# canyagmur/XPoint

Measured on AMD Instinct MI355X. Metric: image-pairs/sec (detect+describe+match) 480x640 optical-thermal, higher is better.
Workload: dtype f32 (dense layers: f32 operands as 2 fp16 terms (operand error <= 2^-23, dropped cross term <= 2^-22: per product <= 2^-21 worst case, ~2^-25 typical), 3 fp16-MFMA partial products, f32 accumulate — GEMMs, implicit-GEMM convolutions and the fused block kernels alike; the deep-stage scan's dt project

## Files before the change

include/xpoint_hip.h:

```cpp
#ifndef XPOINT_HIP_H
#define XPOINT_HIP_H

#include <stddef.h>
#include <stdint.h>

#ifdef __cplusplus
extern "C" {
#endif

int xp_version(void);
const char* xp_last_error(void);
int xp_device_info(int device, int* cu_count, int* wave_size, char* arch, int arch_len);
int xp_knob_count(void);
int xp_knob_info(int index, const char** name, const char** where, const char** what);

int xp_selective_scan_fwd(const float* u, const float* delta, const float* A, const float* B, const float* C,
                          const float* D, const float* delta_bias, float* out, float* last_state,
                          int batch, int dim, int delta_dim, int seqlen, int dstate, int ngroups,
                          int delta_softplus, void* stream);

int xp_selective_scan_fwd_typed(const void* u, const void* delta, const float* A, const void* B, const void* C, const float* D,
                                const float* delta_bias, void* out, float* x_chunks, int itype, int out_float, int batch, int dim,
                                int delta_dim, int seqlen, int dstate, int ngroups, int delta_softplus, void* stream);

// ... 17 lines not shown
int xp_gemm_nt(const float* A, const float* Wt, float* C, const float* bias, const float* scale, const float* shift,
               const float* res, int M, int N, int K, int lda, int ldc, int ldres, int act, void* stream);
int xp_conv3x3_nhwc(const float* x, const float* Wt, float* y, const float* bias, const float* scale,
                    const float* shift, int batch, int Hi, int Wi, int Ci, int Co, int stride, int reflect_pad,
                    int act, void* stream);

size_t xp_split_weights_x3_bytes(int N, int K);
int xp_split_weights_x3(const float* W, void* out, int N, int K, void* stream);
int xp_gemm_nt_x3(const float* A, const void* Wx3, float* C, const float* bias, const float* scale,
                  const float* shift, const float* res, int M, int N, int K, int lda, int ldc, int ldres, int act,
                  void* stream);
int xp_conv3x3_nhwc_x3(const float* x, const void* Wx3, float* y, const float* bias, const float* scale,
                       const float* shift, int batch, int Hi, int Wi, int Ci, int Co, int stride, int reflect_pad,
                       int act, void* stream);
size_t xp_split_weights_h2_bytes(int N, int K);
int xp_split_weights_h2(const float* W, void* out, int N, int K, void* stream);
int xp_gemm_nt_h2(const float* A, const void* Wh2, float* C, const float* bias, const float* scale, const float* shift,
                  const float* res, int M, int N, int K, int lda, int ldc, int ldres, int act, void* stream);
int xp_conv3x3_nhwc_h2(const float* x, const void* Wh2, float* y, const float* bias, const float* scale, const float* shift,
                       int batch, int Hi, int Wi, int Ci, int Co, int stride, int reflect_pad, int act, void* stream);
size_t xp_p32_bytes(int64_t M, int K);
int xp_split_activations_h2(const float* x, void* out_p32, int64_t M, int K, int ldx, void* stream);
int xp_gemm_nt_h2s_applies(int N, int K);
int xp_gemm_nt_h2s(const void* A_p32, const void* Wh2, void* C, int out_fmt, const float* bias, const float* scale, const float* shift,
                   const float* res, int M, int N, int K, int ldc, int ldres, int act, void* stream);
int xp_layernorm_p32(const float* x, void* y_p32, const float* w, const float* b, int64_t rows, int C, float eps, void* stream);
int xp_f32_to_f16(const float* x, void* y, int64_t n, void* stream);
int xp_gemm_nt_f16(const void* A, const void* W, void* C, int c_f32, const float* bias, const float* scale, const float* shift, const void* res,
                   int M, int N, int K, int lda, int ldc, int ldres, int act, void* stream);
int xp_conv3x3_nhwc_f16(const void* x, const void* W, void* y, int y_f32, const float* bias, const float* scale, const float* shift,
                        int batch, int Hi, int Wi, int Ci, int Co, int stride, int reflect_pad, int act, void* stream);

int xp_mlp_fused_f16_supported(int C, int H4);
int xp_mlp_fused_f16(const void* a, void* x, const void* W1, const float* b1, const void* W2, const float* b2, int M, int C, int H4, void* stream);
int xp_ln_mlp_fused_f16(void* x, const float* ln_w, const float* ln_b, float eps, const void* W1, const float* b1, const void* W2, const float* b2,
                        int M, int C, int H4, void* stream);
int xp_ln_proj_f16(const void* x, const float* ln_w, const float* ln_b, float eps, const void* W, void* y, int M, int C, void* stream);
int xp_stem_conv_ln_gelu_f16(const float* img, const float* w9co, const float* bias, const float* ln_w, const float* ln_b, void* y,
                             int batch, int H, int W, int CO, float eps, void* stream);
int xp_layernorm_f16(const void* x, void* y, const float* w, const float* b, int64_t rows, int C, float eps, void* stream);
int xp_dwconv3x3_silu_f16(const void* x, const float* w9c, void* y, float* y_f32_copy, int batch, int H, int W, int C, void* stream);
int xp_depth_to_space_nhwc_f16(const void* x, float* y_f32, void* y_f16, int batch, int H, int W, int C, int bs, int* status, void* stream);
int xp_ss2d_core_f16_wants_f32_copies(int H, int W, int C, int R);
int xp_ss2d_core_fwd_f16(const void* u, const void* xdbl, const float* u_f32, const float* xdbl_f32, const float* wdt, const float* dt_bias,
                         const float* A, const float* Ds, const float* ln_w, const float* ln_b, void* out, float* workspace, size_t workspace_bytes,
                         int batch, int H, int W, int C, int R, int dstate, float eps, void* stream);
size_t xp_f16_weights_bytes(void* ctx);
int xp_prepare_f16_weights(void* ctx, const float* weights, void* w16, size_t w16_bytes, void* stream);
int xp_xpoint_forward_f16(void* ctx, const float* weights, const void* w16, const float* images, int batch, int H, int W, void* workspace,
                          size_t workspace_bytes, float* prob, float* desc_nhwc, float* enc_nhwc, float* logits_nhwc, int* status, void* stream);

int xp_set_dense_products(int n);
int xp_get_dense_products(void);
int xp_set_dense_engine(int engine);
int xp_get_dense_engine(void);
#define XP_DENSE_LAUNCHES 47
int xp_set_dense_override(unsigned long long mask);
unsigned long long xp_get_dense_override(void);
int xp_set_amp_mode(int mode);
int xp_get_amp_mode(void);
int xp_round_f16(const float* x, float* y, int64_t n, void* stream);

int xp_mlp_fused_x3_supported(int C, int hidden);
size_t xp_mlp_fused_x3_pack_bytes(int C, int hidden, int with_proj);
int xp_mlp_fused_x3_pack(const void* W1x3, const void* W2x3, const void* W0x3, void* out, int C, int hidden, void* stream);
int xp_mlp_fused_x3(float* X, const float* T1, const float* ln_w, const float* ln_b, const void* Wpack, const float* b1,
                    const float* b2, int M, int C, int hidden, float eps, void* stream);
size_t xp_mlp_fused_h2_pack_bytes(int C, int hidden, int with_proj);
int xp_mlp_fused_h2_pack(const void* W1h2, const void* W2h2, const void* W0h2, void* out, int C, int hidden, void* stream);
int xp_mlp_fused_h2(float* X, const float* T1, const float* ln_w, const float* ln_b, const void* Wpack, const void* W1h2, const void* W2h2,
                    const void* W0h2, const float* b1, const float* b2, int M, int C, int hidden, float eps, void* stream);
size_t xp_ln_proj_h2_pack_bytes(int C, int N);
int xp_ln_proj_h2_pack(const void* W0h2, void* out, int C, int N, void* stream);
int xp_ln_proj_h2(const float* X, const float* ln_w, const float* ln_b, const void* Wpack, const void* W0h2, float* Out, int M, int C, int N,
                  float eps, void* stream);
size_t xp_ln_proj_x3_pack_bytes(int C, int N);
int xp_ln_proj_x3_pack(const void* W0x3, void* out, int C, int N, void* stream);
int xp_ln_proj_x3(const float* X, const float* ln_w, const float* ln_b, const void* Wpack, float* Out, int M, int C, int N,
                  float eps, void* stream);

int xp_layernorm(const float* x, float* y, const float* w, const float* b, int64_t rows, int C, float eps, int gelu,
                 void* stream);
int xp_dwconv3x3_silu(const float* x, const float* w9c, float* y, int batch, int H, int W, int C, void* stream);
int xp_stem_conv_ln_gelu(const float* img, const float* w9co, const float* bias, const float* ln_w, const float* ln_b,
                         float* y, int batch, int H, int W, int Co, float eps, void* stream);
int xp_depth_to_space_nhwc(const float* x, float* y, int batch, int H, int W, int C, int bs, void* stream);
int xp_softmax_shuffle(const float* logits, float* prob, int batch, int Hc, int Wc, int r, int ld, int mode, void* stream);
int xp_l2norm_rows(const float* x, float* y, int64_t rows, int C, float eps, void* stream);
int xp_nhwc_to_nchw(const float* x, float* y, int batch, int HW, int C, void* stream);
int xp_mul_mask(const float* x, const uint8_t* mask, float* y, int64_t n, void* stream);
int xp_stage_pair_batch(const float* optical, const float* thermal, float* images, const uint8_t* mask_optical,
                        const uint8_t* mask_thermal, uint8_t* masks, int64_t n, void* stream);
int xp_maxpool2_nhwc(const float* x, float* y, int batch, int H, int W, int C, void* stream);
int xp_costvolume_mean(const float* a, const float* b, float* v, int batch, int hw, int C, void* stream);
int xp_ingest_u8(const uint8_t* src, int H0, int W0, int channels, int top, int left, int h, int w,
                 const float* lut256, float* dst, void* stream);
int xp_u8_to_unit_f32(const uint8_t* src, float* dst, int64_t n, void* stream);
int xp_copy_to_mapped_host(const void* src_dev, void* dst_host, size_t bytes, void* stream);

typedef struct xp_model_cfg {
    int embed_dim;
    int n_stages;
    int depths[4];
    int d_state;
    int dt_rank;
    float mlp_ratio;
    int head_channels;
    int desc_size;
    int det_channels;
} xp_model_cfg;

int xp_ctx_create(const xp_model_cfg* cfg, void** ctx);
int xp_ctx_destroy(void* ctx);
int xp_param_count(void* ctx);
size_t xp_weights_numel(void* ctx);
int xp_param_info(void* ctx, int index, char* name, int name_len, size_t* offset, size_t* numel);
int xp_forward_shapes(void* ctx, int batch, int H, int W, int* Hc, int* Wc, int* enc_channels);
size_t xp_forward_workspace_bytes(void* ctx, int batch, int H, int W);
size_t xp_split_weights_bytes(void* ctx);
int xp_prepare_split_weights(void* ctx, const float* weights, void* wsplit, size_t wsplit_bytes, void* stream);
int xp_xpoint_forward(void* ctx, const float* weights, const void* wsplit, const float* images, int batch, int H, int W,
                      void* workspace, size_t workspace_bytes, float* prob, float* desc_nhwc, float* enc_nhwc,
                      float* logits_nhwc, void* stream);
#define XP_STATUS_ENC 1
#define XP_STATUS_PROB 2
#define XP_STATUS_DESC 4
int xp_xpoint_forward_ex(void* ctx, const float* weights, const void* wsplit, const float* images, int batch, int H, int W,
                         void* workspace, size_t workspace_bytes, float* prob, float* desc_nhwc, float* enc_nhwc,
                         float* logits_nhwc, int* status, void* stream);

size_t xp_box_nms_workspace_bytes(int batch, int H, int W, int cap);
int xp_box_nms(const float* prob, float* out, void* workspace, size_t workspace_bytes, int batch, int H, int W,
               float size, float min_prob, float iou, int keep_top_k, int cap, int max_sweeps_async,
               int* converged_host, void* stream);
int xp_box_nms_check(const void* workspace, int batch, int H, int W, int* undecided_tiles, void* stream);

size_t xp_extract_keypoints_workspace_bytes(int batch, int H, int W);
int xp_extract_keypoints(const float* prob, const uint8_t* mask, float thr, int* kp, int* counts, int batch, int H,
                         int W, int cap, void* workspace, size_t workspace_bytes, void* stream);

int xp_sample_descriptors(const int* kp, const int* counts, const float* desc_nhwc, float* out, int batch, int cap,
                          int Hc, int Wc, int D, int H, int W, void* stream);

size_t xp_match_workspace_bytes(int pairs, int cap1, int cap2, int D);
int xp_match_mnn(const float* d1, const float* d2, const int* counts, int cnt_stride, int which1, int which2, int pairs,
                 int cap1, int cap2, int D, int mode, int* idx12, float* dist12, int* idx21, float* dist21,
                 int* match_q, int* match_t, float* match_d, int* match_count, void* workspace, size_t workspace_bytes,
                 void* stream);
int xp_match_knn2(const float* d1, const float* d2, const int* counts, int cnt_stride, int which1, int which2, int pairs, int cap1, int cap2,
                  int D, int* idx2, float* dist2, void* workspace, size_t workspace_bytes, void* stream);
int xp_match_threshold(const float* d1, const float* d2, const int* counts, int cnt_stride, int which1, int which2, int pairs, int cap1, int cap2,
                       int D, double threshold, int* hits, int hit_cap, int* out_pairs, float* out_dist, int* out_count, int out_cap,
                       void* workspace, size_t workspace_bytes, void* stream);
int xp_match_stats(void* workspace, const int* counts, int cnt_stride, int which1, int which2, int pairs, int cap1, int cap2, int D,
                   unsigned long long* out4, void* stream);
int xp_match_cand_cap(void);

int xp_points_min_dist(const double* a, int na, const float* b, int nb, float* out, void* stream);

int xp_gather_match_points(const int* kp, const int* match_q, const int* match_t, const int* match_count, int pairs, int cap,
                           float* src, float* dst, void* stream);
size_t xp_find_homography_workspace_bytes(int pairs);
int xp_find_homography(const float* src, const float* dst, const int* counts, int pairs, int cap, float reproj_thr,
                       int max_iters, unsigned seed, double* H, uint8_t* mask, int* n_inliers, void* workspace,
                       size_t workspace_bytes, void* stream);

// ... 34 lines not shown
```

xpoint_amd/_lib.py:

```python
from __future__ import annotations

import ctypes
import os

_HERE = os.path.dirname(os.path.abspath(__file__))
LIB_PATH = os.environ.get("XP_LIB_PATH") or os.path.join(_HERE, "libxpoint_hip.so")

_lib = None

c_p = ctypes.c_void_p
c_i = ctypes.c_int
c_f = ctypes.c_float
c_l = ctypes.c_int64


class XPointHipError(RuntimeError):
    pass


c_sz = ctypes.c_size_t
_SIGNATURES = {
    "xp_device_info": [c_i, ctypes.POINTER(c_i), ctypes.POINTER(c_i), ctypes.c_char_p, c_i],
    "xp_knob_info": [c_i, ctypes.POINTER(ctypes.c_char_p), ctypes.POINTER(ctypes.c_char_p), ctypes.POINTER(ctypes.c_char_p)],
    "xp_selective_scan_fwd": [c_p] * 9 + [c_i] * 7 + [c_p],
    "xp_selective_scan_fwd_typed": [c_p] * 9 + [c_i] * 9 + [c_p],
    "xp_cross_scan": [c_p, c_p] + [c_i] * 9 + [c_p],
    "xp_cross_merge": [c_p, c_p] + [c_i] * 9 + [c_p],
    "xp_ss2d_core_fwd": [c_p] * 10 + [c_sz] + [c_i] * 6 + [c_f, c_p],
    "xp_ss2d_core_set_mode": [c_i],
    "xp_set_dense_products": [c_i],
    "xp_set_dense_engine": [c_i],
    "xp_set_dense_override": [ctypes.c_uint64],
    "xp_set_amp_mode": [c_i],
    "xp_round_f16": [c_p, c_p, c_l, c_p],
    "xp_gemm_nt": [c_p] * 7 + [c_i] * 7 + [c_p],
    "xp_conv3x3_nhwc": [c_p] * 6 + [c_i] * 8 + [c_p],
    "xp_split_weights_x3": [c_p, c_p, c_i, c_i, c_p],
    "xp_gemm_nt_x3": [c_p] * 7 + [c_i] * 7 + [c_p],
    "xp_conv3x3_nhwc_x3": [c_p] * 6 + [c_i] * 8 + [c_p],
    "xp_split_weights_h2": [c_p, c_p, c_i, c_i, c_p],
    "xp_gemm_nt_h2": [c_p] * 7 + [c_i] * 7 + [c_p],
    "xp_conv3x3_nhwc_h2": [c_p] * 6 + [c_i] * 8 + [c_p],
    "xp_split_activations_h2": [c_p, c_p, c_l, c_i, c_i, c_p],
    "xp_gemm_nt_h2s": [c_p, c_p, c_p, c_i] + [c_p] * 4 + [c_i] * 6 + [c_p],
    "xp_layernorm_p32": [c_p] * 4 + [c_l, c_i, c_f, c_p],
    "xp_ss2d_core_fwd_ex": [c_p] * 9 + [c_i, c_p, c_sz] + [c_i] * 6 + [c_f, c_p],
    "xp_f32_to_f16": [c_p, c_p, c_l, c_p],
    "xp_gemm_nt_f16": [c_p, c_p, c_p, c_i] + [c_p] * 4 + [c_i] * 7 + [c_p],
    "xp_conv3x3_nhwc_f16": [c_p, c_p, c_p, c_i] + [c_p] * 3 + [c_i] * 8 + [c_p],
    "xp_mlp_fused_h2": [c_p] * 10 + [c_i] * 3 + [c_f, c_p],
    "xp_mlp_fused_h2_pack": [c_p] * 4 + [c_i] * 2 + [c_p],
    "xp_ln_proj_h2_pack": [c_p] * 2 + [c_i] * 2 + [c_p],
    "xp_ln_proj_h2": [c_p] * 6 + [c_i] * 3 + [c_f, c_p],
    "xp_mlp_fused_x3": [c_p] * 7 + [c_i] * 3 + [c_f, c_p],
    "xp_mlp_fused_x3_pack": [c_p] * 4 + [c_i] * 2 + [c_p],
    "xp_ln_proj_x3_pack": [c_p] * 2 + [c_i] * 2 + [c_p],
    "xp_ln_proj_x3": [c_p] * 5 + [c_i] * 3 + [c_f, c_p],
    "xp_layernorm": [c_p] * 4 + [c_l, c_i, c_f, c_i, c_p],
    "xp_dwconv3x3_silu": [c_p] * 3 + [c_i] * 4 + [c_p],
    "xp_stem_conv_ln_gelu": [c_p] * 6 + [c_i] * 4 + [c_f, c_p],
    "xp_depth_to_space_nhwc": [c_p] * 2 + [c_i] * 5 + [c_p],
    "xp_softmax_shuffle": [c_p] * 2 + [c_i] * 6 + [c_p],
    "xp_l2norm_rows": [c_p] * 2 + [c_l, c_i, c_f, c_p],
    "xp_nhwc_to_nchw": [c_p] * 2 + [c_i] * 3 + [c_p],
    "xp_mul_mask": [c_p] * 3 + [c_l, c_p],
    "xp_stage_pair_batch": [c_p] * 6 + [c_l, c_p],
    "xp_maxpool2_nhwc": [c_p] * 2 + [c_i] * 4 + [c_p],
    "xp_costvolume_mean": [c_p] * 3 + [c_i] * 3 + [c_p],
    "xp_ingest_u8": [c_p] + [c_i] * 7 + [c_p] * 3,
    "xp_u8_to_unit_f32": [c_p, c_p, c_l, c_p],
    "xp_copy_to_mapped_host": [c_p, c_p, c_sz, c_p],
    "xp_ctx_create": [c_p, ctypes.POINTER(c_p)],
    "xp_ctx_destroy": [c_p],
    "xp_param_info": [c_p, c_i, ctypes.c_char_p, c_i, ctypes.POINTER(c_sz), ctypes.POINTER(c_sz)],
    "xp_forward_shapes": [c_p, c_i, c_i, c_i, ctypes.POINTER(c_i), ctypes.POINTER(c_i), ctypes.POINTER(c_i)],
    "xp_xpoint_forward": [c_p, c_p, c_p, c_p, c_i, c_i, c_i, c_p, c_sz, c_p, c_p, c_p, c_p, c_p],
    "xp_xpoint_forward_ex": [c_p, c_p, c_p, c_p, c_i, c_i, c_i, c_p, c_sz, c_p, c_p, c_p, c_p, c_p, c_p],
    "xp_xpoint_forward_f16": [c_p, c_p, c_p, c_p, c_i, c_i, c_i, c_p, c_sz, c_p, c_p, c_p, c_p, c_p, c_p],
    "xp_prepare_f16_weights": [c_p, c_p, c_p, c_sz, c_p],
    "xp_mlp_fused_f16": [c_p] * 6 + [c_i] * 3 + [c_p],
    "xp_ln_proj_f16": [c_p, c_p, c_p, c_f, c_p, c_p, c_i, c_i, c_p],
    "xp_ln_mlp_fused_f16": [c_p, c_p, c_p, c_f, c_p, c_p, c_p, c_p] + [c_i] * 3 + [c_p],
    "xp_stem_conv_ln_gelu_f16": [c_p] * 6 + [c_i] * 4 + [c_f, c_p],
    "xp_layernorm_f16": [c_p] * 4 + [c_l, c_i, c_f, c_p],
    "xp_dwconv3x3_silu_f16": [c_p] * 4 + [c_i] * 4 + [c_p],
    "xp_depth_to_space_nhwc_f16": [c_p] * 3 + [c_i] * 5 + [c_p, c_p],
    "xp_ss2d_core_fwd_f16": [c_p] * 11 + [c_p, c_sz] + [c_i] * 6 + [c_f, c_p],
    "xp_prepare_split_weights": [c_p, c_p, c_p, c_sz, c_p],
    "xp_box_nms": [c_p, c_p, c_p, c_sz, c_i, c_i, c_i, c_f, c_f, c_f, c_i, c_i, c_i, ctypes.POINTER(c_i), c_p],
    "xp_box_nms_check": [c_p, c_i, c_i, c_i, ctypes.POINTER(c_i), c_p],
    "xp_extract_keypoints": [c_p, c_p, c_f, c_p, c_p, c_i, c_i, c_i, c_i, c_p, c_sz, c_p],
    "xp_sample_descriptors": [c_p] * 4 + [c_i] * 7 + [c_p],
    "xp_match_mnn": [c_p, c_p, c_p] + [c_i] * 8 + [c_p] * 9 + [c_sz, c_p],
    "xp_match_knn2": [c_p, c_p, c_p] + [c_i] * 7 + [c_p, c_p, c_p, c_sz, c_p],
    "xp_match_threshold": [c_p, c_p, c_p] + [c_i] * 7 + [ctypes.c_double, c_p, c_i, c_p, c_p, c_p, c_i, c_p, c_sz, c_p],
    "xp_match_stats": [c_p, c_p] + [c_i] * 7 + [c_p, c_p],
    "xp_points_min_dist": [c_p, c_i, c_p, c_i, c_p, c_p],
    "xp_gather_match_points": [c_p, c_p, c_p, c_p, c_i, c_i, c_p, c_p, c_p],
    "xp_find_homography": [c_p, c_p, c_p, c_i, c_i, c_f, c_i, ctypes.c_uint, c_p, c_p, c_p, c_p, c_sz, c_p],
    "xp_warp_perspective": [c_p, c_p, c_p] + [c_i] * 9 + [c_p],
    "xp_warp_perspective_masked": [c_p, c_p, c_p, c_p] + [c_i] * 9 + [c_p],
    "xp_ha_warp": [c_p] * 3 + [c_i] * 8 + [c_p],
    "xp_ha_valid_mask": [c_p] * 3 + [c_i] * 5 + [c_p],
    "xp_ha_gaussian": [c_p] * 3 + [c_i] * 4 + [c_p],
    "xp_ha_accumulate": [c_p] * 6 + [c_i] * 9 + [c_f, c_p],
    "xp_prof_enable": [c_i],
    "xp_prof_filter": [ctypes.c_char_p],
    "xp_prof_reset": [],
    "xp_prof_count": [],
    "xp_prof_get": [c_i, ctypes.c_char_p, c_i, ctypes.POINTER(ctypes.c_double), ctypes.POINTER(c_i),
                    ctypes.POINTER(ctypes.c_double), ctypes.POINTER(ctypes.c_double)],
}
_SIZE_QUERIES = {
    "xp_knob_count": (c_i, []),
    "xp_weights_numel": (c_sz, [c_p]),
    "xp_param_count": (c_i, [c_p]),
    "xp_forward_workspace_bytes": (c_sz, [c_p, c_i, c_i, c_i]),
    "xp_ss2d_core_workspace_bytes": (c_sz, [c_i] * 4),
    "xp_split_weights_x3_bytes": (c_sz, [c_i] * 2),
    "xp_split_weights_h2_bytes": (c_sz, [c_i] * 2),
    "xp_p32_bytes": (c_sz, [c_l, c_i]),
    "xp_gemm_nt_h2s_applies": (c_i, [c_i, c_i]),
    "xp_ss2d_core_p32_supported": (c_i, [c_i] * 4),
    "xp_split_weights_bytes": (c_sz, [c_p]),
    "xp_f16_weights_bytes": (c_sz, [c_p]),
    "xp_mlp_fused_f16_supported": (c_i, [c_i, c_i]),
    "xp_ss2d_core_f16_wants_f32_copies": (c_i, [c_i] * 4),
    "xp_mlp_fused_x3_supported": (c_i, [c_i, c_i]),
    "xp_get_dense_products": (c_i, []),
    "xp_get_dense_engine": (c_i, []),
    "xp_get_dense_override": (ctypes.c_uint64, []),
    "xp_get_amp_mode": (c_i, []),
    "xp_mlp_fused_x3_pack_bytes": (c_sz, [c_i, c_i, c_i]),
    "xp_mlp_fused_h2_pack_bytes": (c_sz, [c_i, c_i, c_i]),
    "xp_ln_proj_h2_pack_bytes": (c_sz, [c_i, c_i]),
    "xp_ln_proj_x3_pack_bytes": (c_sz, [c_i, c_i]),
    "xp_find_homography_workspace_bytes": (c_sz, [c_i]),
    "xp_box_nms_workspace_bytes": (c_sz, [c_i] * 4),
    "xp_match_workspace_bytes": (c_sz, [c_i] * 4),
    "xp_match_cand_cap": (c_i, []),
    "xp_extract_keypoints_workspace_bytes": (c_sz, [c_i] * 3),
}


def exported_symbols():
    import re
    hdr = os.path.join(_HERE, "..", "include", "xpoint_hip.h")
    txt = open(hdr).read()
    return sorted(set(re.findall(r"\b(xp_[a-z0-9_]+)\s*\(", txt)))


def load():
    global _lib
    if _lib is not None:
        return _lib
    if not os.path.exists(LIB_PATH):
        raise XPointHipError(
            f"{LIB_PATH} not found: build it with `python -m xpoint_amd.build` (hipcc, gfx950). "
            "xpoint_amd has no CPU fallback.")
    import torch
    lib = ctypes.CDLL(LIB_PATH)
    lib.xp_last_error.restype = ctypes.c_char_p
    lib.xp_last_error.argtypes = []
    lib.xp_version.restype = c_i
    for name, argtypes in _SIGNATURES.items():
        fn = getattr(lib, name)
        fn.argtypes = argtypes
        fn.restype = c_i
    for name, (res, argtypes) in _SIZE_QUERIES.items():
        fn = getattr(lib, name)
        fn.argtypes = argtypes
        fn.restype = res
    _lib = lib
    return lib


def check(rc: int, what: str = ""):
    if rc != 0:
        msg = load().xp_last_error().decode("utf-8", "replace")
        raise XPointHipError(f"{what} failed (rc={rc}): {msg}")


def call(name: str, *args):
    lib = load()
    check(getattr(lib, name)(*args), name)


def ptr(t):
    if t is None:
        return None
    assert t.is_cuda and t.is_contiguous(), "xpoint_amd ops need contiguous device tensors"
    return ctypes.c_void_p(t.data_ptr())


def current_stream(device=None):
    import torch
    if device is not None and hasattr(device, "device"):
        device = device.device
    return ctypes.c_void_p(torch.cuda.current_stream(device).cuda_stream)
```

xpoint_amd/csrc/model.cpp:

```cpp
#include <math.h>
#include <stdlib.h>
#include <string.h>

#include <string>
#include <vector>

#include "xp_common.h"
#include "../../include/xpoint_hip.h"

namespace {

struct Param { std::string name; size_t offset; size_t numel; };
struct SplitW { std::string name; size_t src_offset; int N, K; size_t byte_offset, h2_offset, f16_offset; };
struct MlpPack { std::string block; int C, H4; size_t byte_offset, in_offset, h2_offset, h2_in_offset; };

struct Ctx {
    xp_model_cfg cfg;
    int nstages;
    int dims[4], ranks[4];
    std::vector<Param> params;
    std::vector<SplitW> split;
    std::vector<MlpPack> packs;
    size_t total, split_bytes, h2_bytes;
    size_t f16_bytes;
// ... 174 lines not shown

extern "C" size_t xp_forward_workspace_bytes(void* ctx, int batch, int H, int W) {
    if (!ctx) return 0;
    Ctx* c = (Ctx*)ctx; Shapes s;
    if (!shapes_of(*c, batch, H, W, s)) return 0;
    return plan_ws(*c, batch, s).total_floats * sizeof(float);
}

extern "C" size_t xp_split_weights_bytes(void* ctx) { return ctx ? ((Ctx*)ctx)->split_bytes + ((Ctx*)ctx)->h2_bytes : 0; }

#define RUN(call) do { int rc__ = (call); if (rc__ != XP_OK) return rc__; } while (0)

extern "C" int xp_prepare_split_weights(void* ctx, const float* weights, void* wsplit, size_t wsplit_bytes, void* stream) {
    XP_CHECK_ARG(ctx && weights && wsplit, "xp_prepare_split_weights: null pointer");
    Ctx* c = (Ctx*)ctx;
    XP_CHECK_ARG(wsplit_bytes >= c->split_bytes + c->h2_bytes, "xp_prepare_split_weights: buffer too small");
    XP_CHECK_ARG(((uintptr_t)wsplit & 15) == 0, "xp_prepare_split_weights: buffer must be 16-byte aligned");
    for (auto& e : c->split) {
        XP_CHECK_ARG(e.K % 4 == 0, "xp_prepare_split_weights: %s has K = %d, not a multiple of 4", e.name.c_str(), e.K);
        RUN(xp_split_weights_x3(weights + e.src_offset, (char*)wsplit + e.byte_offset, e.N, e.K, stream));
        RUN(xp_split_weights_h2(weights + e.src_offset, (char*)wsplit + c->split_bytes + e.h2_offset, e.N, e.K, stream));
    }
    for (auto& e : c->packs)
        RUN(xp_mlp_fused_x3_pack((char*)wsplit + c->split_off(e.block + "fc1_w"), (char*)wsplit + c->split_off(e.block + "fc2_w"),
                                 (char*)wsplit + c->split_off(e.block + "out_w"), (char*)wsplit + e.byte_offset, e.C, e.H4, stream));
    for (auto& e : c->packs)
        RUN(xp_ln_proj_x3_pack((char*)wsplit + c->split_off(e.block + "in_w"), (char*)wsplit + e.in_offset, e.C, e.C, stream));
    for (auto& e : c->packs) {
        char* w = (char*)wsplit;
        RUN(xp_mlp_fused_h2_pack(w + c->h2_off(e.block + "fc1_w"), w + c->h2_off(e.block + "fc2_w"), w + c->h2_off(e.block + "out_w"),
                                 w + c->split_bytes + e.h2_offset, e.C, e.H4, stream));
        RUN(xp_ln_proj_h2_pack(w + c->h2_off(e.block + "in_w"), w + c->split_bytes + e.h2_in_offset, e.C, e.C, stream));
    }
    return XP_OK;
}

extern "C" int xp_xpoint_forward(void* ctx, const float* weights, const void* wsplit, const float* images, int batch, int H, int W,
                                 void* workspace, size_t workspace_bytes, float* prob, float* desc_nhwc, float* enc_nhwc,
                                 float* logits_nhwc, void* stream) {
    return xp_xpoint_forward_ex(ctx, weights, wsplit, images, batch, H, W, workspace, workspace_bytes, prob, desc_nhwc, enc_nhwc, logits_nhwc,
                                nullptr, stream);
}

extern "C" int xp_xpoint_forward_ex(void* ctx, const float* weights, const void* wsplit, const float* images, int batch, int H, int W,
                                    void* workspace, size_t workspace_bytes, float* prob, float* desc_nhwc, float* enc_nhwc,
                                    float* logits_nhwc, int* status, void* stream) {
    XP_CHECK_ARG(ctx && weights && images && workspace && enc_nhwc, "xp_xpoint_forward: null pointer");
    XP_CHECK_ARG(batch > 0, "xp_xpoint_forward: empty batch");
    Ctx* c = (Ctx*)ctx; Shapes sh;
    XP_CHECK_ARG(shapes_of(*c, batch, H, W, sh), "xp_xpoint_forward: image too small");
    XP_CHECK_ARG(H % 32 == 0 && W % 32 == 0, "xp_xpoint_forward: H and W must be multiples of 32 for the VMamba encoder (got %dx%d)", H, W);
    XP_CHECK_ARG(sh.Hc * 8 == H && sh.Wc * 8 == W, "xp_xpoint_forward: encoder output %dx%d is not 1/8 of the image", sh.Hc, sh.Wc);
    const WsPlan wp = plan_ws(*c, batch, sh);
    XP_CHECK_ARG(workspace_bytes >= wp.total_floats * sizeof(float), "xp_xpoint_forward: workspace too small");
    float* ws = (float*)workspace;
    float *X = ws + wp.X, *T1 = ws + wp.T1, *T2 = ws + wp.T2, *T3 = ws + wp.T3, *HB = ws + wp.HB, *XD = ws + wp.XD, *SS = ws + wp.SS;
    auto P = [&](const std::string& n) -> const float* { return weights + c->off(n); };
    const bool h2 = xp_dense_engine_value() == 1 && xp_dense_products_value() == 6;
    const unsigned long long ovmask = (h2 && !xp_amp_value()) ? xp_dense_override_value() : 0ull;
    auto ov = [&](int id) { return id >= 0 && id < 64 && ((ovmask >> id) & 1ull) != 0; };
    int block_index = 0;
    auto blk = [&]() { const int b = block_index < 7 ? block_index : 7; ++block_index; return 1 + 5 * b; };
    auto gemm = [&](const float* A, const std::string& w, float* C, const float* bias, const float* scale, const float* shift,
                    const float* res, int M, int N, int K, int lda, int ldc, int ldres, int act, int id) -> int {
        if (wsplit && h2 && !ov(id)) return xp_gemm_nt_h2(A, (const char*)wsplit + c->h2_off(w), C, bias, scale, shift, res, M, N, K, lda, ldc, ldres, act, stream);
        if (wsplit) return xp_gemm_nt_x3(A, (const char*)wsplit + c->split_off(w), C, bias, scale, shift, res, M, N, K, lda, ldc, ldres, act, stream);
        return xp_gemm_nt(A, P(w), C, bias, scale, shift, res, M, N, K, lda, ldc, ldres, act, stream);
    };
    auto conv = [&](const float* x, const std::string& w, float* y, const float* bias, const float* scale, const float* shift,
                    int Hi, int Wi, int Ci, int Co, int stride, int reflect, int act, int id) -> int {
        if (wsplit && h2 && !ov(id)) return xp_conv3x3_nhwc_h2(x, (const char*)wsplit + c->h2_off(w), y, bias, scale, shift, batch, Hi, Wi, Ci, Co, stride, reflect, act, stream);
        if (wsplit) return xp_conv3x3_nhwc_x3(x, (const char*)wsplit + c->split_off(w), y, bias, scale, shift, batch, Hi, Wi, Ci, Co, stride, reflect, act, stream);
        return xp_conv3x3_nhwc(x, P(w), y, bias, scale, shift, batch, Hi, Wi, Ci, Co, stride, reflect, act, stream);
    };
    const float eps = 1e-5f;
    const int E = c->cfg.embed_dim;
    static const bool no_fused_mlp = getenv("XP_NO_FUSED_MLP") != nullptr && atoi(getenv("XP_NO_FUSED_MLP")) != 0;
    const bool amp = xp_amp_value() != 0;
    XP_CHECK_ARG(!amp || (wsplit && h2), "xp_xpoint_forward: the mixed-precision class (xp_set_amp_mode) runs on the split-fp16 engine: pass wsplit and "
                 "select xp_set_dense_engine(1) with xp_set_dense_products(6)");
    const bool fuse_mlp = wsplit != nullptr && !no_fused_mlp && !amp;
    static const int fuse_max_c = getenv("XP_FUSE_MAXC") ? atoi(getenv("XP_FUSE_MAXC")) : 1 << 30;
    static const bool fused_x3 = getenv("XP_FUSED_X3") != nullptr && atoi(getenv("XP_FUSED_X3")) != 0;

    RUN(xp_stem_conv_ln_gelu(images, P("stem.w"), P("stem.b"), P("stem.ln_w"), P("stem.ln_b"), HB, batch, H, W, E / 2, eps, stream));
    RUN(conv(HB, "pe2.w", T1, P("pe2.b"), nullptr, nullptr, sh.Hs, sh.Ws, E / 2, E, 2, 0, 0, 0));
    RUN(xp_layernorm(T1, X, P("pe2.ln_w"), P("pe2.ln_b"), sh.M[0], E, eps, 0, stream));

    for (int s = 0; s < c->nstages; ++s) {
        const int C = c->dims[s], R = c->ranks[s], H4 = (int)(C * c->cfg.mlp_ratio);
        const int M = (int)sh.M[s];
        const int XW = 4 * (R + 2);
        for (int j = 0; j < c->cfg.depths[s]; ++j) {
            const std::string b = "s" + std::to_string(s) + ".b" + std::to_string(j) + ".";
            const bool fused_block = fuse_mlp && C <= fuse_max_c && c->pack_off(b) != (size_t)-1;
            const int id0 = blk();
            const bool ring_ok = wsplit && h2 && !amp && !fused_block;
            const bool ring_in = ring_ok && xp_gemm_nt_h2s_applies(C, C) && !ov(id0);
            const bool ring_out = ring_ok && xp_gemm_nt_h2s_applies(C, C) && !ov(id0 + 2) && xp_ss2d_core_p32_supported(sh.H[s], sh.W[s], C, R);
            const bool ring_mlp = ring_ok && xp_gemm_nt_h2s_applies(H4, C) && xp_gemm_nt_h2s_applies(C, H4) && !ov(id0 + 3) && !ov(id0 + 4);
            const bool tail_x3 = ov(id0 + 2) || ov(id0 + 3) || ov(id0 + 4);
            const char* wb = (const char*)wsplit;
            if (fused_block) {
                const char* w = (const char*)wsplit;
                if (h2 && !fused_x3 && !ov(id0)) RUN(xp_ln_proj_h2(X, P(b + "ln1_w"), P(b + "ln1_b"), w + c->h2_pack_off(b, true), w + c->h2_off(b + "in_w"), T2, M, C, C, eps, stream));
                else RUN(xp_ln_proj_x3(X, P(b + "ln1_w"), P(b + "ln1_b"), w + c->in_pack_off(b), T2, M, C, C, eps, stream));
            } else if (ring_in) {
                RUN(xp_layernorm_p32(X, T1, P(b + "ln1_w"), P(b + "ln1_b"), M, C, eps, stream));
                RUN(xp_gemm_nt_h2s(T1, wb + c->h2_off(b + "in_w"), T2, 0, nullptr, nullptr, nullptr, nullptr, M, C, C, C, 0, 0, stream));
            } else {
                RUN(xp_layernorm(X, T1, P(b + "ln1_w"), P(b + "ln1_b"), M, C, eps, 0, stream));
                RUN(gemm(T1, b + "in_w", T2, nullptr, nullptr, nullptr, nullptr, M, C, C, C, C, 0, 0, id0));
            }
            RUN(xp_dwconv3x3_silu(T2, P(b + "dw_w"), T3, batch, sh.H[s], sh.W[s], C, stream));
            RUN(gemm(T3, b + "xproj_w", XD, nullptr, nullptr, nullptr, nullptr, M, XW, C, C, XW, 0, 0, id0 + 1));
            RUN(xp_ss2d_core_fwd_ex(T3, XD, P(b + "dt_w"), P(b + "dt_b"), P(b + "A"), P(b + "D"), P(b + "onorm_w"), P(b + "onorm_b"),
                                    T1, ring_out ? 2 : 0, SS, wp.ss_bytes, batch, sh.H[s], sh.W[s], C, R, 1, eps, stream));
            if (amp) RUN(xp_round_f16(T1, T1, (int64_t)M * C, stream));
            if (fused_block) {
                const char* w = (const char*)wsplit;
                if (h2 && !fused_x3 && !tail_x3) RUN(xp_mlp_fused_h2(X, T1, P(b + "ln2_w"), P(b + "ln2_b"), w + c->h2_pack_off(b, false), w + c->h2_off(b + "fc1_w"), w + c->h2_off(b + "fc2_w"),
                                                         w + c->h2_off(b + "out_w"), P(b + "fc1_b"), P(b + "fc2_b"), M, C, H4, eps, stream));
                else RUN(xp_mlp_fused_x3(X, T1, P(b + "ln2_w"), P(b + "ln2_b"), w + c->pack_off(b), P(b + "fc1_b"), P(b + "fc2_b"), M, C, H4, eps, stream));
                continue;
            }
            if (ring_out) RUN(xp_gemm_nt_h2s(T1, wb + c->h2_off(b + "out_w"), X, 0, nullptr, nullptr, nullptr, X, M, C, C, C, C, 0, stream));
            else RUN(gemm(T1, b + "out_w", X, nullptr, nullptr, nullptr, X, M, C, C, C, C, C, 0, id0 + 2));
            if (ring_mlp) {
                RUN(xp_layernorm_p32(X, T1, P(b + "ln2_w"), P(b + "ln2_b"), M, C, eps, stream));
                RUN(xp_gemm_nt_h2s(T1, wb + c->h2_off(b + "fc1_w"), HB, 2, P(b + "fc1_b"), nullptr, nullptr, nullptr, M, H4, C, H4, 0, 1, stream));
                RUN(xp_gemm_nt_h2s(HB, wb + c->h2_off(b + "fc2_w"), X, 0, P(b + "fc2_b"), nullptr, nullptr, X, M, C, H4, C, C, 0, stream));
                continue;
            }
            RUN(xp_layernorm(X, T1, P(b + "ln2_w"), P(b + "ln2_b"), M, C, eps, 0, stream));
            RUN(gemm(T1, b + "fc1_w", HB, P(b + "fc1_b"), nullptr, nullptr, nullptr, M, H4, C, C, H4, 0, 1, id0 + 3));
            RUN(gemm(HB, b + "fc2_w", X, P(b + "fc2_b"), nullptr, nullptr, X, M, C, H4, H4, C, C, 0, id0 + 4));
        }
        if (s < c->nstages - 1) {
            const std::string d = "s" + std::to_string(s) + ".ds.";
            RUN(conv(X, d + "w", T1, P(d + "b"), nullptr, nullptr, sh.H[s], sh.W[s], C, 2 * C, 2, 0, 0, 41 + s));
            RUN(xp_layernorm(T1, X, P(d + "ln_w"), P(d + "ln_b"), sh.M[s + 1], 2 * C, eps, 0, stream));
        }
    }
    const int L = c->nstages - 1;
    RUN(xp_depth_to_space_nhwc_st(X, enc_nhwc, batch, sh.H[L], sh.W[L], c->dims[L], 4, (wsplit && h2 && !ov(44)) ? 65504.f : INFINITY, status, stream));

    const int EC = enc_channels_of(*c), HC = c->cfg.head_channels, DET = c->cfg.det_channels, DS = c->cfg.desc_size;
    const int Mc = batch * sh.Hc * sh.Wc;
    if (prob || logits_nhwc || desc_nhwc) {
        RUN(conv(enc_nhwc, "head.w", HB, P("head.b"), P("head.scale"), P("head.shift"), sh.Hc, sh.Wc, EC, 2 * HC, 1, 1, 2, 44));
    }
    if (prob || logits_nhwc) {
        float* lg = logits_nhwc ? logits_nhwc : T2;
        RUN(gemm(HB, "det2.w", lg, P("det2.b"), P("det2.scale"), P("det2.shift"), nullptr, Mc, DET, HC, 2 * HC, DET, 0, 0, 45));
        if (prob) RUN(xp_softmax_shuffle_st(lg, prob, batch, sh.Hc, sh.Wc, 8, DET, 0, status, stream));
    }
    if (desc_nhwc) {
        RUN(gemm(HB + HC, "desc2.w", T1, P("desc2.b"), P("desc2.scale"), P("desc2.shift"), nullptr, Mc, DS, HC, 2 * HC, DS, 0, 0, 46));
        RUN(xp_l2norm_rows_st(T1, desc_nhwc, Mc, DS, 1e-12f, status, stream));
    }
    return XP_OK;
}


extern "C" size_t xp_f16_weights_bytes(void* ctx) { return ctx ? ((Ctx*)ctx)->f16_bytes : 0; }

extern "C" int xp_prepare_f16_weights(void* ctx, const float* weights, void* w16, size_t w16_bytes, void* stream) {
    XP_CHECK_ARG(ctx && weights && w16, "xp_prepare_f16_weights: null pointer");
    Ctx* c = (Ctx*)ctx;
    XP_CHECK_ARG(w16_bytes >= c->f16_bytes, "xp_prepare_f16_weights: buffer too small");
    XP_CHECK_ARG(((uintptr_t)w16 & 255) == 0, "xp_prepare_f16_weights: buffer must be 256-byte aligned");
    for (auto& e : c->split) {
        XP_CHECK_ARG(e.K % 8 == 0, "xp_prepare_f16_weights: %s has K = %d, not a multiple of 8", e.name.c_str(), e.K);
        RUN(xp_f32_to_f16(weights + e.src_offset, (char*)w16 + e.f16_offset, (int64_t)e.N * e.K, stream));
    }
    return XP_OK;
}

extern "C" int xp_xpoint_forward_f16(void* ctx, const float* weights, const void* w16, const float* images, int batch, int H, int W,
                                     void* workspace, size_t workspace_bytes, float* prob, float* desc_nhwc, float* enc_nhwc,
                                     float* logits_nhwc, int* status, void* stream) {
    XP_CHECK_ARG(ctx && weights && w16 && images && workspace && enc_nhwc, "xp_xpoint_forward_f16: null pointer");
    XP_CHECK_ARG(batch > 0, "xp_xpoint_forward_f16: empty batch");
    Ctx* c = (Ctx*)ctx; Shapes sh;
    XP_CHECK_ARG(shapes_of(*c, batch, H, W, sh), "xp_xpoint_forward_f16: image too small");
    XP_CHECK_ARG(H % 32 == 0 && W % 32 == 0, "xp_xpoint_forward_f16: H and W must be multiples of 32 for the VMamba encoder (got %dx%d)", H, W);
    XP_CHECK_ARG(sh.Hc * 8 == H && sh.Wc * 8 == W, "xp_xpoint_forward_f16: encoder output %dx%d is not 1/8 of the image", sh.Hc, sh.Wc);
    XP_CHECK_ARG(c->cfg.embed_dim % 16 == 0, "xp_xpoint_forward_f16: embed_dim must be a multiple of 16");
    const WsPlan wp = plan_ws(*c, batch, sh);
    XP_CHECK_ARG(workspace_bytes >= wp.total_floats * sizeof(float), "xp_xpoint_forward_f16: workspace too small");
    float* ws = (float*)workspace;
    typedef unsigned short h16;
    h16 *X = (h16*)(ws + wp.X), *T1 = (h16*)(ws + wp.T1), *T2 = (h16*)(ws + wp.T2), *T3 = (h16*)(ws + wp.T3), *HB = (h16*)(ws + wp.HB), *XD = (h16*)(ws + wp.XD);
    float* SS = ws + wp.SS;
    auto P = [&](const std::string& n) -> const float* { return weights + c->off(n); };
    auto WH = [&](const std::string& n) -> const void* { return (const char*)w16 + c->f16_off(n); };
    auto gemm = [&](const void* A, const std::string& w, void* C, int c_f32, const float* bias, const float* scale, const float* shift,
                    const void* res, int M, int N, int K, int lda, int ldc, int ldres, int act) -> int {
// ... 76 lines not shown
```

xpoint_amd/csrc/xp_knobs.h:

```cpp
#pragma once

struct XpKnob { const char* name; const char* where; const char* what; };

static const XpKnob kXpKnobs[] = {
    {"XP_DENSE_ENGINE", "api.cpp", "initial value of xp_set_dense_engine: h2 (default) | x3"},
    {"XP_DENSE_PRODUCTS", "api.cpp", "initial value of xp_set_dense_products: 6 (default) | 3 | 1"},
    {"XP_RING", "gemm_ring.hip", "0: keep every layer on the round-4 GEMM kernels (default 1: ring engine for N, K >= 256 layers of the split class)"},
    {"XP_RING_TILE", "gemm_ring.hip", "force the ring tile: 0 = 256x256, 1 = 256x128, 2 = 128x128"},
    {"XP_H2P", "gemm_h2p.hip", "ping-pong split-fp16 GEMM: 0 off, 1 (default) K >= 768 and N >= 384, 2 widened"},
    {"XP_H2_ENGINE", "gemm_h2.hip", "rs | lds: force the row-stationary / tile variant of the split-fp16 GEMM"},
    {"XP_H2_TILE", "gemm_h2.hip", "force the split-fp16 tile (0..4)"},
    {"XP_H2_NO64", "gemm_h2.hip", "64x128 tile rule: 0 old, 1 never, 2 (default) only below 128 tiles"},
    {"XP_H2_NGROUP", "gemm_h2.hip", "column tiles per group of the tile order (0 = N-fastest)"},
    {"XP_X3_TILE", "gemm_x3.hip", "force the split-bf16 tile"},
    {"XP_GEMM_STAGGER", "gemm.hip", "exact-f32 GEMM: start-up delay (cycles) of the second workgroup slot of every CU"},
    {"XP_GEMM_STAMPS", "gemm.hip", "exact-f32 GEMM: s_memtime stamps per workgroup (debug)"},
    {"XP_F16_TILE", "gemm_f16.hip", "force the fp16-class tile (0..5)"},
    {"XP_F16_BK", "gemm_f16.hip", "force the fp16-class slab depth: 32 | 64"},
    {"XP_NO_FUSED_MLP", "model.cpp", "1: stages 0-1 as separate launches instead of xp_ln_proj + xp_mlp_fused"},
    {"XP_FUSE_MAXC", "model.cpp", "blocks wider than this many channels run unfused"},
    {"XP_FUSED_X3", "model.cpp", "1: fused block kernels on the x3 planes under the h2 engine"},
    {"XP_NO_LN_PROJ_F16", "model.cpp", "fp16 class: LayerNorm and in_proj as two launches"},
    {"XP_NO_FUSED_MLP_F16", "model.cpp", "fp16 class: 1 two-GEMM MLP everywhere, 2 fused MLP behind a separate LayerNorm"},
    {"XP_MLP_TAIL", "mlp_fused.hip", "0: no separate 4-wave launch for a last round less than half full (C = 192)"},
    {"XP_MLP_NW8", "mlp_fused.hip", "1: 8-wave workgroups in the x3 fused tail (C <= 96)"},
    {"XP_MLP_H2_NW4", "mlp_fused.hip", "1: 4-wave workgroups in the h2 fused tail at C = 192"},
    {"XP_SS2D_SEQ", "ss2d.hip", "0 / 1: force the chunked / sequential form of the fused SS2D core (also xp_ss2d_core_set_mode)"},
    {"XP_SS2D_SEQ_MAXL", "ss2d.hip", "L bound of the automatic choice of the sequential form (default 8192)"},
    {"XP_SS2D_SEQ_V1", "ss2d.hip", "1: first sequential kernel (dt projection on the vector ALU)"},
    {"XP_SS2D_SEQ_NW", "ss2d.hip", "waves per route of the pipelined sequential kernel: 1 | 2 | 4"},
    {"XP_SS2D_TBUDGET", "ss2d.hip", "chunk-length budget of the chunked passes (default 6144 pixel-channels)"},
    {"XP_SS2D_T", "ss2d.hip", "chunk length per channel count, e.g. \"96:32,192:16,384:16\""},
    {"XP_SS2D_THREADS", "ss2d.hip", "threads per workgroup of the chunked passes (default 192)"},
    {"XP_SCAN_V1", "selective_scan.hip", "force the first d_state = 1 operator-boundary scan kernel"},
    {"XP_SCAN_V2", "selective_scan.hip", "force the second d_state = 1 operator-boundary scan kernel"},
    {"XP_SCAN_OLD_GEN", "selective_scan.hip", "1: the round-1 generic-N operator-boundary scan kernel"},
    {"XP_NMS_SCHED", "postproc.hip", "NMS local-iteration schedule"},
    {"XP_NMS_SWEEP", "postproc.hip", "NMS sweep count"},
    {"XP_NMS_WIDE_ROUNDS", "postproc.hip", "wide suppression rounds ahead of the NMS finisher"},
    {"XP_PROF_SHAPES", "*.hip", "1: per-shape tags in the HIP-event breakdown (xp_prof_*)"},
    {"XP_GEMM_MODE", "models.py / bench.py", "default gemm_mode of models.XPoint: h2 | x3 | f32 | x2 | bf16 | amp16 | amp16f"},
    {"XP_HONOR_MIXED_PRECISION", "models.py", "1: take the precision class from the config's mixed_precision flag"},
    {"XP_LIB_PATH", "_lib.py", "load another build of libxpoint_hip.so"},
    {"XP_EXTRA_HIPCC_FLAGS", "build.py", "extra hipcc flags of `python -m xpoint_amd.build`"},
    {"XP_D2H_COPY_ENGINE", "predict.py", "1: result lists to the host through the runtime's copy engines instead of xp_copy_to_mapped_host (A/B)"},
    {"XP_C5_HEAD_STREAM", "streaming.py", "caller: the RegNet head of the streaming step on the caller's stream (round-4 placement) instead of the detection / matching stream (A/B)"},
    {"XP_RANK_CPUS", "affinity.py", "pin every rank to this cpulist instead of its GPU's NUMA CPUs"},
    {"XP_CPU_THREADS", "bench.py", "threads of the CPU baseline"},
    {"XP_BENCH_DEPTH", "bench.py", "steps in flight of the alternating-encoder schedule (default 3)"},
    {"XP_BENCH_NO_PIN", "bench.py", "1: do not pin the rank to its GPU's NUMA CPUs"},
    {"XP_BENCH_NO_RCCL", "bench.py", "1: world 1 without a live RCCL communicator"},
    {"XP_BENCH_REHEARSE_ON_ONE_GPU", "bench.py", "1: --gpus N on a 1-GPU box: the N ranks share GPU 0, collectives over gloo (code-path rehearsal of the N-rank line; rates meaningless)"},
    {"XP_BENCH_PCIE_PARTS", "bench.py", "1: print the parts of the streaming loop (profiles/r5_streaming_parts.txt)"},
};
static const int kXpKnobCount = (int)(sizeof(kXpKnobs) / sizeof(kXpKnobs[0]));
```

Measured before the change: 1769.

## Fuse depthwise conv+SiLU with x_proj GEMM into one h2 MFMA kernel

```diff
diff --git a/include/xpoint_hip.h b/include/xpoint_hip.h
--- a/include/xpoint_hip.h
+++ b/include/xpoint_hip.h
@@ -123,6 +123,9 @@
 int xp_layernorm(const float* x, float* y, const float* w, const float* b, int64_t rows, int C, float eps, int gelu,
                  void* stream);
 int xp_dwconv3x3_silu(const float* x, const float* w9c, float* y, int batch, int H, int W, int C, void* stream);
+int xp_dwconv_xproj_h2_supported(int C, int N);
+int xp_dwconv_silu_xproj_h2(const float* x, const float* w9c, const void* Wh2, float* y, float* xd, int batch, int H, int W, int C, int N,
+                            void* stream);
 int xp_stem_conv_ln_gelu(const float* img, const float* w9co, const float* bias, const float* ln_w, const float* ln_b,
                          float* y, int batch, int H, int W, int Co, float eps, void* stream);
 int xp_depth_to_space_nhwc(const float* x, float* y, int batch, int H, int W, int C, int bs, void* stream);
diff --git a/xpoint_amd/_lib.py b/xpoint_amd/_lib.py
--- a/xpoint_amd/_lib.py
+++ b/xpoint_amd/_lib.py
@@ -58,6 +58,7 @@
     "xp_ln_proj_x3": [c_p] * 5 + [c_i] * 3 + [c_f, c_p],
     "xp_layernorm": [c_p] * 4 + [c_l, c_i, c_f, c_i, c_p],
     "xp_dwconv3x3_silu": [c_p] * 3 + [c_i] * 4 + [c_p],
+    "xp_dwconv_silu_xproj_h2": [c_p] * 5 + [c_i] * 5 + [c_p],
     "xp_stem_conv_ln_gelu": [c_p] * 6 + [c_i] * 4 + [c_f, c_p],
     "xp_depth_to_space_nhwc": [c_p] * 2 + [c_i] * 5 + [c_p],
     "xp_softmax_shuffle": [c_p] * 2 + [c_i] * 6 + [c_p],
@@ -127,6 +128,7 @@
     "xp_mlp_fused_f16_supported": (c_i, [c_i, c_i]),
     "xp_ss2d_core_f16_wants_f32_copies": (c_i, [c_i] * 4),
     "xp_mlp_fused_x3_supported": (c_i, [c_i, c_i]),
+    "xp_dwconv_xproj_h2_supported": (c_i, [c_i, c_i]),
     "xp_get_dense_products": (c_i, []),
     "xp_get_dense_engine": (c_i, []),
     "xp_get_dense_override": (ctypes.c_uint64, []),
diff --git a/xpoint_amd/csrc/dwconv_xproj.hip b/xpoint_amd/csrc/dwconv_xproj.hip
--- /dev/null
+++ b/xpoint_amd/csrc/dwconv_xproj.hip
@@ -0,0 +1,186 @@
+#include <stdlib.h>
+
+#include <string>
+
+#include "gemm_h2_core.h"
+
+namespace {
+
+constexpr int DX_TH = 4, DX_TW = 32;
+constexpr int DX_HR = DX_TH + 2, DX_HC = DX_TW + 2;
+constexpr int DX_HALO_PIX = DX_HR * DX_HC;
+constexpr int DX_HALO_Q = DX_HALO_PIX * 8;
+constexpr int DX_HALO_LD = (DX_HALO_Q + 255) / 256;
+constexpr int DX_HALO_BYTES = DX_HALO_PIX * 128;
+constexpr int DX_A_BYTES = DX_TH * DX_TW * H2_ROWB;
+constexpr int DX_MAX_C = 192;
+
+template <int TN>
+__global__ __launch_bounds__(256, 3) void dwconv_xproj_h2_kernel(const float* __restrict__ x, const float* __restrict__ dw, const uint4* __restrict__ wt,
+                                                              const float* __restrict__ wscale, float* __restrict__ y, float* __restrict__ xd,
+                                                              int B, int H, int W, int C, int N) {
+    __shared__ __align__(16) unsigned char lds_halo[DX_HALO_BYTES];
+    __shared__ __align__(16) unsigned char lds_a[DX_A_BYTES];
+    __shared__ __align__(16) unsigned char lds_dw[9 * DX_MAX_C * 4];
+    const int tid = threadIdx.x, lane = tid & 63, wave = tid >> 6;
+    const int fr = lane & 31, fh = lane >> 5;
+    const int TWn = (W + DX_TW - 1) / DX_TW, THn = (H + DX_TH - 1) / DX_TH;
+    const unsigned nb = gridDim.x, xcd = blockIdx.x & 7, slot = blockIdx.x >> 3, q8 = nb >> 3, r8 = nb & 7;
+    const int tile = (int)((xcd < r8 ? xcd * (q8 + 1) : r8 * (q8 + 1) + (xcd - r8) * q8) + slot);
+    const int tw = tile % TWn, th = (tile / TWn) % THn, b = tile / (TWn * THn);
+    const int h0 = th * DX_TH, w0 = tw * DX_TW;
+    const int64_t img = (int64_t)b * H * W;
+
+    const int nslab = C / H2_BK;
+    const int nslab2 = (nslab + 1) & ~1;
+    const int C4 = C >> 2;
+
+    float4 hv[DX_HALO_LD];
+    auto load_halo = [&](int t) {
+#pragma unroll
+        for (int s = 0; s < DX_HALO_LD; ++s) {
+            const int i = tid + s * 256;
+            const int pix = i >> 3, q = i & 7;
+            const int hr = pix / DX_HC, hc = pix - hr * DX_HC;
+            const int ih = h0 - 1 + hr, iw = w0 - 1 + hc;
+            const bool ok = i < DX_HALO_Q && ih >= 0 && ih < H && iw >= 0 && iw < W;
+            hv[s] = ok ? reinterpret_cast<const float4*>(x)[(img + (int64_t)ih * W + iw) * C4 + t * 8 + q] : make_float4(0.f, 0.f, 0.f, 0.f);
+        }
+    };
+    auto store_halo = [&]() {
+#pragma unroll
+        for (int s = 0; s < DX_HALO_LD; ++s) {
+            const int i = tid + s * 256;
+            if (s + 1 < DX_HALO_LD || i < DX_HALO_Q) *reinterpret_cast<float4*>(lds_halo + i * 16) = hv[s];
+        }
+    };
+
+    const int dq = tid & 7, dc = tid >> 3;
+    f32x16 acc[TN];
+#pragma unroll
+    for (int j = 0; j < TN; ++j)
+#pragma unroll
+        for (int r = 0; r < 16; ++r) acc[j][r] = 0.f;
+    const int a_frag = (wave * 32 + fr) * H2_ROWB + 16 * fh;
+    typedef unsigned ubits4 __attribute__((ext_vector_type(4)));
+    auto slab_mfmas = [&](int t, bool zero_a) {
+        const int tb = t < nslab ? t : nslab - 1;
+#pragma unroll
+        for (int ks = 0; ks < 2; ++ks) {
+            f16x8_t a0, a1, bf[2][TN];
+            if (zero_a) {
+                a0 = __builtin_bit_cast(f16x8_t, ubits4{0u, 0u, 0u, 0u}); a1 = a0;
+            } else {
+                a0 = *reinterpret_cast<const f16x8_t*>(lds_a + a_frag + ks * 32);
+                a1 = *reinterpret_cast<const f16x8_t*>(lds_a + a_frag + 64 + ks * 32);
+            }
+#pragma unroll
+            for (int pl = 0; pl < 2; ++pl)
+#pragma unroll
+                for (int j = 0; j < TN; ++j) {
+                    const int n = j * 32 + fr;
+                    bf[pl][j] = __builtin_bit_cast(f16x8_t, wt[((int64_t)tb * N + (n < N ? n : 0)) * H2_SLAB_UNITS + pl * 4 + ks * 2 + fh]);
+                }
+#pragma unroll
+            for (int j = 0; j < TN; ++j) acc[j] = __builtin_amdgcn_mfma_f32_32x32x16_f16(a1, bf[0][j], acc[j], 0, 0, 0);
+#pragma unroll
+            for (int j = 0; j < TN; ++j) acc[j] = __builtin_amdgcn_mfma_f32_32x32x16_f16(a0, bf[1][j], acc[j], 0, 0, 0);
+#pragma unroll
+            for (int j = 0; j < TN; ++j) acc[j] = __builtin_amdgcn_mfma_f32_32x32x16_f16(a0, bf[0][j], acc[j], 0, 0, 0);
+        }
+    };
+
+    for (int i = tid; i < 9 * C4; i += 256) reinterpret_cast<float4*>(lds_dw)[i] = reinterpret_cast<const float4*>(dw)[i];
+    load_halo(0);
+    for (int t = 0; t < nslab; ++t) {
+        store_halo();
+        __syncthreads();
+        {
+            const int c = t * H2_BK + dq * 4;
+            float4 wv[9];
+#pragma unroll
+            for (int k = 0; k < 9; ++k) wv[k] = *reinterpret_cast<const float4*>(lds_dw + (k * C + c) * 4);
+            if (t + 1 < nslab) load_halo(t + 1);
+            float4 a[DX_TH];
+#pragma unroll
+            for (int r = 0; r < DX_TH; ++r) a[r] = make_float4(0.f, 0.f, 0.f, 0.f);
+#pragma unroll
+            for (int ir = 0; ir < DX_HR; ++ir) {
+                const int ih = h0 + ir - 1;
+                if (ih < 0 || ih >= H) continue;
+                float4 col[3];
+#pragma unroll
+                for (int cx = 0; cx < 3; ++cx) col[cx] = *reinterpret_cast<const float4*>(lds_halo + ((ir * DX_HC + dc + cx) * 8 + dq) * 16);
+#pragma unroll
+                for (int r = 0; r < DX_TH; ++r) {
+                    const int kh = ir - r;
+                    if (kh < 0 || kh > 2) continue;
+#pragma unroll
+                    for (int kw = 0; kw < 3; ++kw) {
+                        const int iw = w0 + dc + kw - 1;
+                        if (iw < 0 || iw >= W) continue;
+                        const float4 xin = col[kw], wk = wv[kh * 3 + kw];
+                        a[r].x = fmaf(xin.x, wk.x, a[r].x); a[r].y = fmaf(xin.y, wk.y, a[r].y);
+                        a[r].z = fmaf(xin.z, wk.z, a[r].z); a[r].w = fmaf(xin.w, wk.w, a[r].w);
+                    }
+                }
+            }
+            const int ow = w0 + dc;
+#pragma unroll
+            for (int r = 0; r < DX_TH; ++r) {
+                float4 o = a[r];
+                o.x = xp_silu(o.x); o.y = xp_silu(o.y); o.z = xp_silu(o.z); o.w = xp_silu(o.w);
+                if (h0 + r < H && ow < W) reinterpret_cast<float4*>(y)[(img + (int64_t)(h0 + r) * W + ow) * C4 + (c >> 2)] = o;
+                uint2 p0, p1;
+                h2_split4(o, p0, p1);
+                unsigned char* dst = lds_a + (r * DX_TW + dc) * H2_ROWB + dq * 8;
+                *reinterpret_cast<uint2*>(dst) = p0;
+                *reinterpret_cast<uint2*>(dst + 64) = p1;
+            }
+        }
+        __syncthreads();
+        slab_mfmas(t, false);
+    }
+    if (nslab2 != nslab) slab_mfmas(nslab, true);
+
+    const int oh = h0 + wave;
+#pragma unroll
+    for (int j = 0; j < TN; ++j) {
+        const int col = j * 32 + fr;
+        const bool cok = col < N;
+        const float ws = wscale[cok ? col : 0];
+        const float bi = 0.f, sc = 1.f, sh = 0.f;
+#pragma unroll
+        for (int r = 0; r < 16; ++r) {
+            const int ow = w0 + (r & 3) + 8 * (r >> 2) + 4 * fh;
+            float v = acc[j][r] * ws + bi;
+            v = v * sc + sh;
+            const float o = 0.f + v;
+            if (cok && oh < H && ow < W) xd[(img + (int64_t)oh * W + ow) * N + col] = o;
+        }
+    }
+}
+
+}
+
+extern "C" int xp_dwconv_xproj_h2_supported(int C, int N) { return C > 0 && C % H2_BK == 0 && C <= DX_MAX_C && N > 0 && N <= 64 && N % 4 == 0; }
+
+extern "C" int xp_dwconv_silu_xproj_h2(const float* x, const float* w9c, const void* Wh2, float* y, float* xd, int batch, int H, int W, int C, int N,
+                                       void* stream) {
+    XP_CHECK_ARG(x && w9c && Wh2 && y && xd, "xp_dwconv_silu_xproj_h2: null pointer");
+    XP_CHECK_ARG(batch > 0 && H > 0 && W > 0, "xp_dwconv_silu_xproj_h2: bad shape %d x %d x %d", batch, H, W);
+    XP_CHECK_ARG(xp_dwconv_xproj_h2_supported(C, N), "xp_dwconv_silu_xproj_h2: needs C %% 32 == 0, C <= 192 and N <= 64, N %% 4 == 0 (got C %d, N %d)", C, N);
+    XP_CHECK_ARG(!xp_amp_value(), "xp_dwconv_silu_xproj_h2: the mixed-precision class keeps the two-launch form");
+    const int nslab = C / H2_BK;
+    const float* wscale = reinterpret_cast<const float*>(reinterpret_cast<const char*>(Wh2) + (size_t)N * nslab * H2_SLAB_UNITS * 16);
+    const int64_t tiles = (int64_t)batch * ((H + DX_TH - 1) / DX_TH) * ((W + DX_TW - 1) / DX_TW);
+    XP_CHECK_ARG(tiles < (1ll << 31), "xp_dwconv_silu_xproj_h2: too many tiles");
+    const hipStream_t s = (hipStream_t)stream;
+    const double M = (double)batch * H * W;
+    XpProfScope prof(("dwconv_xproj_h2_c" + std::to_string(C)).c_str(), s, 22.0 * M * C + 2.0 * M * N * C,
+                     4.0 * (2.0 * M * C + M * N + 10.0 * C + (double)N * C));
+    if (N <= 32) hipLaunchKernelGGL((dwconv_xproj_h2_kernel<1>), dim3((unsigned)tiles), dim3(256), 0, s, x, w9c, (const uint4*)Wh2, wscale, y, xd, batch, H, W, C, N);
+    else hipLaunchKernelGGL((dwconv_xproj_h2_kernel<2>), dim3((unsigned)tiles), dim3(256), 0, s, x, w9c, (const uint4*)Wh2, wscale, y, xd, batch, H, W, C, N);
+    XP_LAUNCH_CHECK();
+    return XP_OK;
+}
diff --git a/xpoint_amd/csrc/model.cpp b/xpoint_amd/csrc/model.cpp
--- a/xpoint_amd/csrc/model.cpp
+++ b/xpoint_amd/csrc/model.cpp
@@ -280,6 +280,7 @@
     const bool fuse_mlp = wsplit != nullptr && !no_fused_mlp && !amp;
     static const int fuse_max_c = getenv("XP_FUSE_MAXC") ? atoi(getenv("XP_FUSE_MAXC")) : 1 << 30;
     static const bool fused_x3 = getenv("XP_FUSED_X3") != nullptr && atoi(getenv("XP_FUSED_X3")) != 0;
+    static const int no_fused_glue = getenv("XP_NO_FUSED_GLUE") ? atoi(getenv("XP_NO_FUSED_GLUE")) : 0;
 
     RUN(xp_stem_conv_ln_gelu(images, P("stem.w"), P("stem.b"), P("stem.ln_w"), P("stem.ln_b"), HB, batch, H, W, E / 2, eps, stream));
     RUN(conv(HB, "pe2.w", T1, P("pe2.b"), nullptr, nullptr, sh.Hs, sh.Ws, E / 2, E, 2, 0, 0, 0));
@@ -310,8 +311,12 @@
                 RUN(xp_layernorm(X, T1, P(b + "ln1_w"), P(b + "ln1_b"), M, C, eps, 0, stream));
                 RUN(gemm(T1, b + "in_w", T2, nullptr, nullptr, nullptr, nullptr, M, C, C, C, C, 0, 0, id0));
             }
-            RUN(xp_dwconv3x3_silu(T2, P(b + "dw_w"), T3, batch, sh.H[s], sh.W[s], C, stream));
-            RUN(gemm(T3, b + "xproj_w", XD, nullptr, nullptr, nullptr, nullptr, M, XW, C, C, XW, 0, 0, id0 + 1));
+            if (fused_block && !(no_fused_glue & 2) && wsplit && h2 && !ov(id0 + 1) && xp_dwconv_xproj_h2_supported(C, XW)) {
+                RUN(xp_dwconv_silu_xproj_h2(T2, P(b + "dw_w"), (const char*)wsplit + c->h2_off(b + "xproj_w"), T3, XD, batch, sh.H[s], sh.W[s], C, XW, stream));
+            } else {
+                RUN(xp_dwconv3x3_silu(T2, P(b + "dw_w"), T3, batch, sh.H[s], sh.W[s], C, stream));
+                RUN(gemm(T3, b + "xproj_w", XD, nullptr, nullptr, nullptr, nullptr, M, XW, C, C, XW, 0, 0, id0 + 1));
+            }
             RUN(xp_ss2d_core_fwd_ex(T3, XD, P(b + "dt_w"), P(b + "dt_b"), P(b + "A"), P(b + "D"), P(b + "onorm_w"), P(b + "onorm_b"),
                                     T1, ring_out ? 2 : 0, SS, wp.ss_bytes, batch, sh.H[s], sh.W[s], C, R, 1, eps, stream));
             if (amp) RUN(xp_round_f16(T1, T1, (int64_t)M * C, stream));
diff --git a/xpoint_amd/csrc/xp_knobs.h b/xpoint_amd/csrc/xp_knobs.h
--- a/xpoint_amd/csrc/xp_knobs.h
+++ b/xpoint_amd/csrc/xp_knobs.h
@@ -20,6 +20,7 @@
     {"XP_NO_FUSED_MLP", "model.cpp", "1: stages 0-1 as separate launches instead of xp_ln_proj + xp_mlp_fused"},
     {"XP_FUSE_MAXC", "model.cpp", "blocks wider than this many channels run unfused"},
     {"XP_FUSED_X3", "model.cpp", "1: fused block kernels on the x3 planes under the h2 engine"},
+    {"XP_NO_FUSED_GLUE", "model.cpp", "bit mask: 2 = depthwise conv + SiLU and x_proj of the fused-block stages as two launches instead of xp_dwconv_silu_xproj_h2"},
     {"XP_NO_LN_PROJ_F16", "model.cpp", "fp16 class: LayerNorm and in_proj as two launches"},
     {"XP_NO_FUSED_MLP_F16", "model.cpp", "fp16 class: 1 two-GEMM MLP everywhere, 2 fused MLP behind a separate LayerNorm"},
     {"XP_MLP_TAIL", "mlp_fused.hip", "0: no separate 4-wave launch for a last round less than half full (C = 192)"},
```

Result: no change. 1775, median of 6 (+0.3%).
